# bhavyageethika/multimodal_autonomous_driving_perception_and_planning

Hardware: AMD Instinct MI355X
Metric: end-to-end frames/sec (1280x720 synthetic) (higher is better)
Workload: dtype f64; 1 GPU; config4: 64 stream(s)/GPU x 1-frame window per step, 1280x720, simulated detection + IoU tracker + 6-state KF + 21-candidate planner, one launch per step, up to 4 consecutive steps in flight; streams_per_gpu=64, window=1, graph=False, taggers=False, allgather_track_tables=False, fused_step=True, overlapped_steps=4, steps_per_library_call=8, parallelism=stream-sharded x1

## Files before the change

### include/avhot.h

```cpp
#ifndef AVHOT_H
#define AVHOT_H

#include <stddef.h>
#include <stdint.h>

#ifdef __cplusplus
extern "C" {
#endif

#define AV_VERSION 102

enum {
    AV_OK = 0,
    AV_EINVAL = -1,
    AV_EHIP = -2,
    AV_ENODEV = -3,
    AV_ESTATE = -4,
    AV_ENOMEM = -5
};

typedef struct av_ctx av_ctx;
typedef void* av_stream_t;

int av_version(void);
// ... 73 lines not shown
int av_pack_tracks(av_ctx* ctx, av_stream_t stream, int n_streams, int n_frames, int tcap, int frame_lo, int n_sel,
                   int stream0, int frame0, const av_track_row* snap, const int32_t* snap_n, const int32_t* frame_count, void* wire);

int av_comm_unique_id(void* id128);
int av_comm_create(av_ctx* ctx, const void* id128, int rank, int world, void** comm);
int av_comm_destroy(void* comm);
int av_allgather_tracks(av_ctx* ctx, void* comm, av_stream_t stream, const void* send, void* recv, size_t bytes_per_rank);

typedef struct {
    double dt;
    double process_noise;
    double measurement_noise;
} av_kf_cfg;

#define AV_KF_STATE_DOUBLES 48
#define AV_VSTATE_DOUBLES 12
int av_kf_reset(av_ctx* ctx, av_stream_t stream, int n_streams, double* kf_state);
int av_kf_step(av_ctx* ctx, av_stream_t stream, const av_kf_cfg* cfg, int n_streams, int n_frames,
               const double* z, const uint8_t* mode, double* kf_state, double* out_state,
               double* plan_state);

typedef struct {
    double planning_horizon;
    double dt;
    int32_t num_samples;
    int32_t reserved;
    double w_lateral, w_velocity, w_acceleration, w_curvature;
} av_planner_cfg;

#define AV_WP_DOUBLES 6
int av_planner_configure(av_ctx* ctx, const av_planner_cfg* cfg);
int av_planner_dims(const av_ctx* ctx, int* n_points, int* n_candidates);
int av_planner_launch_shape(int n_points, int n_candidates, int n_states, int extra, int32_t out[4]);
int av_planner_plan(av_ctx* ctx, av_stream_t stream, int n_states, const double* state,
                    const double* ref_path, int n_ref, const double* obstacles, int n_obs,
                    double* waypoints, double* cost, int32_t* order);

int av_planner_plan_each(av_ctx* ctx, av_stream_t stream, int n_states, const double* state,
                         const double* ref_path, const int32_t* n_ref, int rcap, int ref_stride,
                         const double* obstacles, const int32_t* n_obs, int ocap,
                         double* waypoints, double* cost, int32_t* order);

int av_planner_plan_moving(av_ctx* ctx, av_stream_t stream, int n_states, const double* state,
                           const double* ref_path, const int32_t* n_ref, int rcap, int ref_stride,
                           const double* obstacles, const int32_t* n_obs, int ocap,
                           double* waypoints, double* cost, int32_t* order);

typedef struct {
    double x_center, x_scale;
    double y_far, y_scale;
    double radius[16];
} av_obstacle_cfg;
int av_track_obstacles(av_ctx* ctx, av_stream_t stream, const av_obstacle_cfg* cfg, int n_states, int tcap,
                       const av_track_row* snap, const int32_t* snap_n, const double* plan_state,
                       int ocap, double* obstacles, int32_t* n_obs);
int av_track_obstacles_moving(av_ctx* ctx, av_stream_t stream, const av_obstacle_cfg* cfg, double frame_rate, int n_states,
                              int tcap, const av_track_row* snap, const int32_t* snap_n, const double* plan_state,
                              int ocap, double* obstacles, int32_t* n_obs);

int av_dets_to_tracker(av_ctx* ctx, av_stream_t stream, int n_frames, int max_det, const int32_t* src_n,
                       const float* src_box, const float* src_conf, const int32_t* src_cls, const int32_t* class_map,
                       int n_map, int dcap, int32_t* det_n, int32_t* det_box, int32_t* det_cls, double* det_conf,
                       int32_t* dropped);

int av_lane_paths(av_ctx* ctx, av_stream_t stream, const av_obstacle_cfg* cfg, int n_streams, int h, int w, int n_points,
                  const double* poly, const int32_t* pts, const int32_t* info, const double* plan_state, int ref_stride,
// ... 224 lines not shown
```

### multimodal_autonomous_driving_perception_and_planning_amd/_native.py

```python
import ctypes as C
import os

_HERE = os.path.dirname(os.path.abspath(__file__))
LIB_PATH = os.path.join(_HERE, "libavhot.so")

c_i32p = C.POINTER(C.c_int32)
c_f64p = C.POINTER(C.c_double)
vp = C.c_void_p


class TrackerCfg(C.Structure):
    _fields_ = [("iou_threshold", C.c_double), ("max_age", C.c_int32), ("min_hits", C.c_int32),
                ("trajectory_length", C.c_int32)]


class KfCfg(C.Structure):
    _fields_ = [("dt", C.c_double), ("process_noise", C.c_double), ("measurement_noise", C.c_double)]


class PlannerCfg(C.Structure):
    _fields_ = [("planning_horizon", C.c_double), ("dt", C.c_double), ("num_samples", C.c_int32),
                ("reserved", C.c_int32), ("w_lateral", C.c_double), ("w_velocity", C.c_double),
                ("w_acceleration", C.c_double), ("w_curvature", C.c_double)]

# ... 69 lines not shown
    ("av_side_stream", C.c_int, [vp, C.POINTER(vp)]),
    ("av_fork", C.c_int, [vp, vp]),
    ("av_join", C.c_int, [vp, vp]),
    ("av_graph_begin", C.c_int, [vp, vp]),
    ("av_graph_end", C.c_int, [vp, vp, C.POINTER(C.c_int)]),
    ("av_graph_launch", C.c_int, [vp, C.c_int, vp]),
    ("av_graph_destroy", C.c_int, [vp, C.c_int]),
    ("av_event_create", C.c_int, [C.POINTER(vp)]),
    ("av_event_destroy", C.c_int, [vp]),
    ("av_event_record", C.c_int, [vp, vp]),
    ("av_event_elapsed_ms", C.c_int, [vp, vp, C.POINTER(C.c_float)]),
    ("av_stream_sync", C.c_int, [vp]),
    ("av_stream_sync_spin", C.c_int, [vp]),
    ("av_host_alloc", C.c_int, [C.POINTER(vp), C.c_size_t]),
    ("av_host_free", C.c_int, [vp]),
    ("av_copy_h2d", C.c_int, [vp, vp, C.c_size_t, vp]),
    ("av_copy_d2h", C.c_int, [vp, vp, C.c_size_t, vp, C.c_int]),
    ("av_simdet_generate", C.c_int, [vp, vp, C.c_int, C.c_int, C.c_int, C.c_int, C.c_int, vp, vp, vp, vp, vp, vp]),
    ("av_tracker_state_bytes", C.c_size_t, [C.c_int, C.c_int]),
    ("av_tracker_reset", C.c_int, [vp, vp, C.c_int, C.c_int, C.c_int, vp]),
    ("av_tracker_update", C.c_int, [vp, vp, C.POINTER(TrackerCfg), C.c_int, C.c_int, C.c_int, vp, vp, vp, vp,
                                    C.c_int, vp, vp, vp, vp]),
    ("av_wire_table_bytes", C.c_size_t, [C.c_int]),
    ("av_pack_tracks", C.c_int, [vp, vp, C.c_int, C.c_int, C.c_int, C.c_int, C.c_int, C.c_int, C.c_int, vp, vp, vp, vp]),
    ("av_comm_unique_id", C.c_int, [vp]),
    ("av_comm_create", C.c_int, [vp, vp, C.c_int, C.c_int, C.POINTER(vp)]),
    ("av_comm_destroy", C.c_int, [vp]),
    ("av_allgather_tracks", C.c_int, [vp, vp, vp, vp, vp, C.c_size_t]),
    ("av_kf_reset", C.c_int, [vp, vp, C.c_int, vp]),
    ("av_kf_step", C.c_int, [vp, vp, C.POINTER(KfCfg), C.c_int, C.c_int, vp, vp, vp, vp, vp]),
    ("av_planner_configure", C.c_int, [vp, C.POINTER(PlannerCfg)]),
    ("av_planner_dims", C.c_int, [vp, C.POINTER(C.c_int), C.POINTER(C.c_int)]),
    ("av_planner_launch_shape", C.c_int, [C.c_int, C.c_int, C.c_int, C.c_int, c_i32p]),
    ("av_planner_plan", C.c_int, [vp, vp, C.c_int, vp, vp, C.c_int, vp, C.c_int, vp, vp, vp]),
    ("av_planner_plan_each", C.c_int, [vp, vp, C.c_int, vp, vp, vp, C.c_int, C.c_int, vp, vp, C.c_int, vp, vp, vp]),
    ("av_track_obstacles", C.c_int, [vp, vp, C.POINTER(ObstacleCfg), C.c_int, C.c_int, vp, vp, vp, C.c_int, vp, vp]),
    ("av_planner_plan_moving", C.c_int, [vp, vp, C.c_int, vp, vp, vp, C.c_int, C.c_int, vp, vp, C.c_int, vp, vp, vp]),
    ("av_track_obstacles_moving", C.c_int, [vp, vp, C.POINTER(ObstacleCfg), C.c_double, C.c_int, C.c_int, vp, vp, vp, C.c_int, vp,
                                            vp]),
    ("av_dets_to_tracker", C.c_int, [vp, vp, C.c_int, C.c_int, vp, vp, vp, vp, vp, C.c_int, C.c_int, vp, vp, vp, vp, vp]),
    ("av_lane_paths", C.c_int, [vp, vp, C.POINTER(ObstacleCfg), C.c_int, C.c_int, C.c_int, C.c_int, vp, vp, vp, vp, C.c_int,
                                C.c_int, vp, vp, vp]),
    ("av_hot_step", C.c_int, [vp, vp, C.POINTER(TrackerCfg), C.POINTER(KfCfg)] + [C.c_int] * 5 + [vp] * 17 + [vp, C.c_int, C.c_int]),
    ("av_hot_step_fits", C.c_int, [vp, C.c_int, C.c_int, C.c_int, C.c_int]),
    ("av_hot_steps_seq", C.c_int, [vp, C.c_int, vp, C.POINTER(TrackerCfg), C.POINTER(KfCfg)] + [C.c_int] * 5 + [vp] * 7 +
     [C.c_int, C.c_int, vp, C.c_int, C.c_int]),
    ("av_hot_step_seq", C.c_int, [vp, vp, C.POINTER(TrackerCfg), C.POINTER(KfCfg)] + [C.c_int] * 5 + [vp] * 17 +
     [vp, C.c_int, C.c_int, vp, C.c_int, C.c_int]),
    ("av_planner_generate", C.c_int, [vp, vp, C.c_int, vp, vp, vp, vp]),
    ("av_planner_evaluate", C.c_int, [vp, vp, C.c_int, C.c_int, vp, vp, C.c_int, vp, C.c_int, vp]),
    ("av_planner_evaluate_moving", C.c_int, [vp, vp, C.c_int, C.c_int, vp, vp, C.c_int, vp, C.c_int, vp]),
    ("av_lane_workspace_bytes", C.c_size_t, [C.c_int, C.c_int, C.c_int, C.c_int]),
    ("av_lane_workspace_init", C.c_int, [vp, vp, C.c_int, C.c_int, C.c_int, C.c_int, vp]),
    ("av_lane_workspace_view", C.c_int, [C.c_int, C.c_int, C.c_int, C.c_int, C.c_int, C.POINTER(C.c_size_t),
                                         C.POINTER(C.c_size_t)]),
    ("av_raster_draw", C.c_int, [vp, vp, C.c_int, C.c_int, C.c_int, vp, vp, C.c_int, vp, vp, C.c_int]),
    ("av_bev_prim_cap", C.c_int, [vp, C.c_int, C.c_int]),
    ("av_bev_build", C.c_int, [vp, vp, vp, C.c_int, C.c_int, C.c_int, C.c_int, C.c_int, vp, vp, vp, vp, vp, vp, vp, C.c_int, vp]),
    ("av_i420_to_bgr", C.c_int, [vp, vp, C.c_int, C.c_int, C.c_int, vp, vp]),
    ("av_resize_into", C.c_int, [vp, vp, vp, C.c_int, C.c_int, vp, C.c_int, C.c_int, C.c_int, C.c_int]),
    ("av_synth_frames", C.c_int, [vp, vp, C.c_int, C.c_int, C.c_int, C.c_int, C.c_int, vp]),
    ("av_maneuver_reset", C.c_int, [vp, vp, C.c_int, vp]),
    ("av_interaction_state_bytes", C.c_size_t, [C.c_int]),
    ("av_interaction_reset", C.c_int, [vp, vp, C.c_int, C.c_int, vp]),
    ("av_interaction_detect", C.c_int, [vp, vp, vp, C.c_int, C.c_int, C.c_int, vp, vp, vp, vp, vp, vp, vp, vp]),
    ("av_maneuver_detect", C.c_int, [vp, vp, C.c_int, C.c_int, vp, vp, vp, vp]),
# ... 151 lines not shown
```

### multimodal_autonomous_driving_perception_and_planning_amd/csrc/planner.hip

```cpp
#include "common.h"

#include <cmath>



namespace {

struct PlanParams {
    int n, n_lat, C;
    double dt, H;
    double w_lat, w_vel, w_acc, w_curv;
    const double *t, *alpha, *q, *dtd, *lat;
    double atq[20];
};

static const double ATAN_Q[20] = {
    -0x1.5555555555549p-2, 0x1.99999999979b9p-3,  -0x1.24924923e22b4p-3, 0x1.c71c718e5a102p-4,
    -0x1.745d120df88fbp-4, 0x1.3b1362fc35ab5p-4,  -0x1.110deef367776p-4, 0x1.e1b3c8d50e91fp-5,
    -0x1.ae2c7119eb922p-5, 0x1.81fdd2525246ap-5,  -0x1.56daf4786fd80p-5, 0x1.2575526b2309ap-5,
    -0x1.d168e01adf666p-6, 0x1.462cc26bda000p-6,  -0x1.8055065b73333p-7, 0x1.693bd6b79999ap-8,
    -0x1.fdf4e15cccccdp-10, 0x1.f224118000000p-12, -0x1.2568700000000p-14, 0x1.2ed799999999ap-18,
};

__device__ __forceinline__ double atan2_fast(double y, double x, const double (&Q)[20]) {
// ... 63 lines not shown
    tile[(size_t)(n - 1) * 6 + 2] = n > 1 ? tile[(size_t)(n - 2) * 6 + 2] : h0;
}
__device__ __forceinline__ double ref_path_term(double w_lat, const double* ref, int n_ref, double x, double y) {
    double md = INFINITY;
    for (int r = 0; r < n_ref; ++r) {
        const double dx = ref[2 * r] - x, dy = ref[2 * r + 1] - y;
        const double dd = sqrt(dx * dx + dy * dy);
        md = dd < md ? dd : md;
    }
    return w_lat * (md * md);
}
template <bool MOVING>
__device__ __forceinline__ void add_obstacle_penalty(double& sum, const double* o, double x, double y, double tw) {
    double ox = o[0], oy = o[1];
    const double rad = o[2];
    if constexpr (MOVING) ox = ox + o[3] * tw, oy = oy + o[4] * tw;
    const double ex = x - ox, ey = y - oy;
    const double dist = sqrt(ex * ex + ey * ey);
    if (dist < rad * 2.0) sum = sum + 1000.0 * (rad * 2.0 - dist);
    else if (dist < rad * 4.0) sum = sum + 10.0 / (dist - rad + 0.1);
}
__device__ __forceinline__ void rank_and_store(const double* cc, int C, int c, int f, double* __restrict__ cost,
                                               int32_t* __restrict__ order) {
    const double mine = cc[c];
    int rank = 0;
    for (int o2 = 0; o2 < C; ++o2) {
        const double v = cc[o2];
        rank += (v < mine || (v == mine && o2 < c)) ? 1 : 0;
    }
    cost[(size_t)f * C + c] = mine;
    order[(size_t)f * C + rank] = c;
}

struct PlanNoHook {
    __device__ __forceinline__ void operator()(int) const {}
};

struct PlanLists {
    const double* ref; int n_ref;
    const double* obs; int n_obs;
};
struct PlanShared {
    static constexpr int OSTRIDE = 3;
    static constexpr bool MOVING = false;
    const double* ref; int n_ref;
    const double* obs; int n_obs;
    __device__ __forceinline__ PlanLists at(int) const { return PlanLists{ref, n_ref, obs, n_obs}; }
    __device__ __forceinline__ bool has_ref(int) const { return n_ref > 0; }
};
template <int OS>
struct PlanEachT {
    static constexpr int OSTRIDE = OS;
    static constexpr bool MOVING = OS == 5;
    const double* ref; const int32_t* n_ref;
    const double* obs; const int32_t* n_obs;
    int rcap, ref_stride, ocap;
    __device__ __forceinline__ int path_points(int pth) const {
        const int k = n_ref[pth] > rcap ? rcap : n_ref[pth];
        return k < 2 ? 0 : k;
    }
    __device__ __forceinline__ bool has_ref(int f) const { return ref && path_points(f / ref_stride) > 0; }
    __device__ __forceinline__ PlanLists at(int f) const {
        f = __builtin_amdgcn_readfirstlane(f);
        PlanLists l{nullptr, 0, nullptr, 0};
        if (ref) {
            const int pth = f / ref_stride;
            l.n_ref = path_points(pth);
            l.ref = ref + (size_t)pth * rcap * 2;
        }
        if (obs) {
            const int k = n_obs[f];
            l.n_obs = k < 0 ? 0 : (k > ocap ? ocap : k);
            l.obs = obs + (size_t)f * ocap * OS;
        }
        return l;
    }
};
using PlanEach = PlanEachT<3>;
using PlanEachMoving = PlanEachT<5>;

template <int G, int NW, class Hook = PlanNoHook, class Lists = PlanShared>
__device__ __forceinline__ void plan_block_lists(const PlanParams& p, int f0, int n_states, const double* __restrict__ state,
                                                 const Lists lists, double* __restrict__ wp, double* __restrict__ cost,
                                                 int32_t* __restrict__ order, double* sm, int state_f0 = -1, int rot = 0,
                                                 Hook after1 = Hook()) {
    const int n = p.n, C = p.C;
    const int sd = state_f0 < 0 ? 0 : state_f0 - f0;
    double* vs = sm;
    double* base = vs + (size_t)G * 3 * n * 2;
    double* trig = base + even_up(G * 3 * 3);
    double* costs = trig + G * 8;
    double* stage_all = costs + 3 * even_up(G * C);
    const int CS = even_up(G * C);

    const int tid = threadIdx.x, lane = tid & 63;
    double* stage = stage_all + (size_t)(tid >> 6) * n * 6;
    const int wid = ((tid >> 6) + NW - rot) % NW;
    constexpr int P = G * 3;
    static_assert(NW >= 2, "the heading terms take the last wave");

    auto bcast = [&](double x, int i) {
        const unsigned lo = (unsigned)__builtin_amdgcn_readlane((int)(unsigned)__double_as_longlong(x), i);
        const unsigned hi = (unsigned)__builtin_amdgcn_readlane((int)(unsigned)((unsigned long long)__double_as_longlong(x) >> 32), i);
        return __longlong_as_double((long long)(((unsigned long long)hi << 32) | lo));
    };
    auto terms = [&](double v0, double dv, int i, double& v, double& vdt, double& velt, double& acct) {
        v = blend_velocity(v0, dv, p.alpha[i]);
        vdt = v * p.dt;
        velt = velocity_term(p.w_vel, v);
        acct = 0.0;
        if (i > 0)
            acct = acceleration_term(p.w_acc, v, blend_velocity(v0, dv, p.alpha[i - 1]), p.dtd[i]);
    };
    auto cost_chains = [&](double velt, double acct, unsigned long long hasm, double* b) {
        double sv = 0.0;
#pragma unroll
        for (int i = 0; i < 64; ++i)
            if (i < n) sv = sv + bcast(velt, i);
        double run = sv, sa = 0.0;
#pragma unroll
        for (int i = 1; i < 64; ++i)
            if (i < n && ((hasm >> i) & 1ull)) {
                const double term = bcast(acct, i);
                run = run + term, sa = sa + term;
            }
        if (lane == 0) b[0] = sv, b[1] = sa, b[2] = run;
    };

    const bool fast = n <= 64 && P <= NW;
    double k_velt = 0.0, k_acct = 0.0;
    unsigned long long k_has = 0;
    bool k_live = false;
    if (fast) {
        if (wid < P) {
            const int g = wid / 3, k = wid - g * 3, f = f0 + g;
            if (f < n_states) {
                const double v0 = state[(size_t)(f + sd) * 4 + 3];
                const double dv = target_speed(k) - v0;
                double* o = vs + ((size_t)(g * 3 + k) * n) * 2;
                double v = 0.0, vdt = 0.0;
                bool has = false;
                if (lane < n) terms(v0, dv, lane, v, vdt, k_velt, k_acct), has = lane > 0 && p.dtd[lane] > 0.0;
                k_has = __ballot(has), k_live = true;
                double sacc = 0.0, my_s = 0.0;
#pragma unroll
                for (int i = 1; i < 64; ++i)
                    if (i < n) {
                        sacc = sacc + bcast(vdt, i);
                        my_s = lane == i ? sacc : my_s;
                    }
                if (lane < n) o[2 * lane] = v, o[2 * lane + 1] = my_s;
            }
        }
    } else {
        for (int pr = wid; pr < P; pr += NW) {
            const int g = pr / 3, k = pr - g * 3, f = f0 + g;
            if (f >= n_states) continue;
            const double v0 = state[(size_t)(f + sd) * 4 + 3];
            const double dv = target_speed(k) - v0;
            double* o = vs + ((size_t)(g * 3 + k) * n) * 2;
            double* b = base + (g * 3 + k) * 3;
            double* tv = stage;
            for (int i = lane; i < n; i += 64) {
                double v, vdt, velt, acct;
                terms(v0, dv, i, v, vdt, velt, acct);
                o[2 * i] = v, tv[i] = vdt, tv[n + i] = velt, tv[2 * n + i] = acct;
            }
            wave_lds_fence();
            if (lane == 0) {
                double sacc = 0.0, sv = 0.0;
                o[1] = 0.0;
                sv = sv + tv[n];
                for (int i = 1; i < n; ++i) {
                    sacc = sacc + tv[i];
                    o[2 * i + 1] = sacc;
                    sv = sv + tv[n + i];
                }
                double run = sv, sa = 0.0;
                for (int i = 1; i < n; ++i) {
                    if (p.dtd[i] > 0.0) {
                        const double term = tv[2 * n + i];
                        run = run + term, sa = sa + term;
                    }
                }
                b[0] = sv, b[1] = sa, b[2] = run;
            }
            wave_lds_fence();
        }
    }
    if (wid == NW - 1 && lane < 2 * G) {
        const int g = lane >> 1, f = f0 + g;
        if (f < n_states) {
            const double h0 = state[(size_t)(f + sd) * 4 + 2];
            double* tg = trig + g * 8;
            double sn, cs;
            if (lane & 1) {
                sincos(h0 + 1.5707963267948966, &sn, &cs);
                tg[4] = cs, tg[5] = sn;
            } else {
                sincos(h0, &sn, &cs);
                tg[0] = state[(size_t)(f + sd) * 4 + 0], tg[1] = state[(size_t)(f + sd) * 4 + 1];
                tg[2] = cs, tg[3] = sn, tg[6] = h0;
            }
        }
    }
    __syncthreads();
    if (k_live) cost_chains(k_velt, k_acct, k_has, base + wid * 3);
    after1(wid);

    const double q_l = lane < n ? p.q[lane] : 0.0, q_l1 = lane + 1 < n ? p.q[lane + 1] : 0.0, t_l = lane < n ? p.t[lane] : 0.0;
    for (int j = fast ? (wid - P % NW + NW) % NW : wid; j < G * C; j += NW) {
        const int g = j / C, c = j - g * C, f = f0 + g;
        if (f >= n_states) continue;
        const PlanLists ls = lists.at(f);
        const double* ref = ls.ref;
        const double* obs = ls.obs;
        const int n_ref = ls.n_ref, n_obs = ls.n_obs;
        const bool extra = n_ref > 0 || n_obs > 0;
        const int li = c / 3, k = c - li * 3;
        const double df = p.lat[li];
        const double* tg = trig + g * 8;
        const PlanFrame fr{tg[0], tg[1], tg[2], tg[3], tg[4], tg[5]};
        const double h0 = tg[6];
        const double* o = vs + ((size_t)(g * 3 + k) * n) * 2;

        for (int i = lane; i < n; i += 64) {
            const double v = o[2 * i], s = o[2 * i + 1];
            const bool first = i == lane;
            double x, y, hd = 0.0;
            fr.point(s, df * (first ? q_l : p.q[i]), x, y);
            if (i < n - 1) {
                double x1, y1;
                fr.point(o[2 * i + 3], df * (first ? q_l1 : p.q[i + 1]), x1, y1);
                hd = atan2_fast(y1 - y, x1 - x, p.atq);
            }
            double* w = stage + (size_t)i * 6;
            w[0] = x, w[1] = y, w[2] = hd, w[3] = v, w[4] = first ? t_l : p.t[i], w[5] = 0.0;
        }
        wave_lds_fence();
        double lat_sum = 0.0, curv_sum = 0.0, obs_sum = 0.0;
        for (int i = lane; i < n; i += 64) {
            double* w = stage + (size_t)i * 6;
            double curv = 0.0;
            if (i > 0 && i < n - 1) w[5] = curv = tile_curvature(stage, i, p.dt);
            curv_sum += p.w_curv * (curv * curv);
            const double x = w[0], y = w[1];
            if (n_ref > 0) lat_sum += ref_path_term(p.w_lat, ref, n_ref, x, y);
            for (int q = 0; q < n_obs; ++q)
                add_obstacle_penalty<Lists::MOVING>(obs_sum, obs + Lists::OSTRIDE * q, x, y, w[4]);
        }
        wave_lds_fence();
        if (lane == 0) tile_last_heading(stage, n, h0);
        curv_sum = wave_sum_dpp(curv_sum);
        if (extra) lat_sum = wave_sum_dpp(lat_sum), obs_sum = wave_sum_dpp(obs_sum);
        if (lane == 0) costs[g * C + c] = lat_sum, costs[CS + g * C + c] = curv_sum, costs[2 * CS + g * C + c] = obs_sum;
        wave_lds_fence();
        if (wp) {
            const double2* src = reinterpret_cast<const double2*>(stage);
            double2* dst = reinterpret_cast<double2*>(wp + ((size_t)f * C + c) * n * 6);
            for (int q = lane; q < n * 3; q += 64) dst[q] = src[q];
        }
        wave_lds_fence();
    }
    __syncthreads();

    for (int idx = tid; idx < G * C; idx += NW * 64) {
        const int g = idx / C, c = idx - g * C, k = c % 3;
        const double* b = base + (g * 3 + k) * 3;
        const bool with_ref = lists.has_ref(f0 + g < n_states ? f0 + g : f0);
        const double va = with_ref ? (costs[idx] + b[0]) + b[1] : b[2];
        const double total = (va + costs[CS + idx]) + costs[2 * CS + idx];
        costs[idx] = total;
    }
    __syncthreads();
    for (int idx = tid; idx < G * C; idx += NW * 64) {
        const int g = idx / C, c = idx - g * C, f = f0 + g;
        if (f >= n_states) continue;
        rank_and_store(costs + g * C, C, c, f, cost, order);
    }
}

template <int G, int NW, class Hook = PlanNoHook>
__device__ __forceinline__ void plan_block(const PlanParams& p, int f0, int n_states, const double* state, const double* ref, int n_ref,
                                           const double* obs, int n_obs, double* wp, double* cost, int32_t* order, double* sm,
                                           int state_f0 = -1, int rot = 0, Hook after1 = Hook()) {
    plan_block_lists<G, NW, Hook, PlanShared>(p, f0, n_states, state, PlanShared{ref, n_ref, obs, n_obs}, wp, cost, order, sm, state_f0,
                                              rot, after1);
}

template <int G, int NW, class Lists = PlanShared>
__global__ void __launch_bounds__(NW * 64) planner_kernel(PlanParams p, int n_states, const double* __restrict__ state, Lists lists,
                                                          double* __restrict__ wp, double* __restrict__ cost,
                                                          int32_t* __restrict__ order) {
    extern __shared__ __attribute__((aligned(16))) double sm[];
    plan_block_lists<G, NW, PlanNoHook, Lists>(p, blockIdx.x * G, n_states, state, lists, wp, cost, order, sm);
}

template <int FPW, bool EXTRA, class Lists = PlanShared>
__global__ void __launch_bounds__(256) planner_wave_kernel(PlanParams p, int n_states,
                                                           const double* __restrict__ state, Lists lists,
                                                           double* __restrict__ wp, double* __restrict__ cost,
                                                           int32_t* __restrict__ order) {
    extern __shared__ __attribute__((aligned(16))) double sm[];
    const int n = p.n, C = p.C;
    const int lane = threadIdx.x & 63, wid = threadIdx.x >> 6;
    double* vs = sm + wid * wave_lds_doubles(FPW, n, C);
    double* stage = vs + (size_t)FPW * 3 * n * 2;
    double* costs = stage + RING_DOUBLES;
    double* base = costs + even_up(FPW * C);
    double* trig = base + FPW * 3 * 4;
    const long long gw = (long long)blockIdx.x * 4 + wid;
    const long long f0l = gw * FPW;
    if (f0l >= n_states) return;
    const int f0 = (int)f0l;
    const int nf = (n_states - f0) < FPW ? (n_states - f0) : FPW;

    const bool in = lane < n;
    const int li_c = in ? lane : n - 1;
    const int ln_c = (lane + 1 < n) ? lane + 1 : n - 1;
    const int lp_c = li_c > 0 ? li_c - 1 : 0;
    const double q_i = p.q[li_c], q_n = p.q[ln_c], t_i = p.t[li_c];
    const double al_i = p.alpha[li_c], al_p = p.alpha[lp_c], dtd_i = p.dtd[li_c];
    const double lat_l = p.lat[lane < p.n_lat ? lane : 0];
    double st_x[FPW], st_y[FPW], st_h[FPW], st_v[FPW];
#pragma unroll
    for (int g = 0; g < FPW; ++g) {
        const double4 sv4 = reinterpret_cast<const double4*>(state)[f0 + (g < nf ? g : 0)];
        st_x[g] = sv4.x, st_y[g] = sv4.y, st_h[g] = sv4.z, st_v[g] = sv4.w;
// ... 387 lines not shown
        lat[nl - 1] = 3.5;
    }
    AV_HIP(hipSetDevice(ctx->device));
    if (ctx->d_ptab) {
        AV_HIP(hipFree(ctx->d_ptab));
        ctx->d_ptab = nullptr;
    }
    AV_HIP(hipMalloc(&ctx->d_ptab, tab.size() * sizeof(double)));
    AV_HIP(hipMemcpy(ctx->d_ptab, tab.data(), tab.size() * sizeof(double), hipMemcpyHostToDevice));
    ctx->pcfg = *cfg;
    ctx->n_points = n, ctx->n_lat = nl, ctx->n_cand = 3 * nl;
    ctx->planner_ready = true;
    return AV_OK;
}

int av_planner_dims(const av_ctx* ctx, int* n_points, int* n_candidates) {
    AV_REQUIRE(ctx && n_points && n_candidates, AV_EINVAL, "av_planner_dims: null argument");
    AV_REQUIRE(ctx->planner_ready, AV_ESTATE, "av_planner_dims: call av_planner_configure first");
    *n_points = ctx->n_points, *n_candidates = ctx->n_cand;
    return AV_OK;
}

int av_planner_launch_shape(int n_points, int n_candidates, int n_states, int extra, int32_t out[4]) {
    AV_REQUIRE(out, AV_EINVAL, "av_planner_launch_shape: null argument");
    AV_REQUIRE(n_points >= 1 && n_points <= 256 && n_candidates >= 3 && n_candidates <= 192 && n_candidates % 3 == 0, AV_EINVAL,
               "av_planner_launch_shape: %d waypoints, %d candidates: not a configuration av_planner_configure accepts", n_points,
               n_candidates);
    AV_REQUIRE(n_states > 0, AV_EINVAL, "av_planner_launch_shape: n_states must be > 0");
    const PlanLaunch<PlanShared> l = planner_plan<PlanShared>(n_points, n_candidates, n_states, extra != 0);
    out[0] = l.inst->wave, out[1] = l.inst->G, out[2] = l.inst->NW, out[3] = (int32_t)l.lds;
    return AV_OK;
}

int av_planner_plan(av_ctx* ctx, av_stream_t stream, int n_states, const double* state, const double* ref_path,
                    int n_ref, const double* obstacles, int n_obs, double* waypoints, double* cost, int32_t* order) {
    AV_REQUIRE(ctx && state && cost && order, AV_EINVAL, "av_planner_plan: null argument");
    AV_REQUIRE(ctx->planner_ready, AV_ESTATE, "av_planner_plan: call av_planner_configure first");
    AV_REQUIRE(n_states > 0, AV_EINVAL, "av_planner_plan: n_states must be > 0");
    AV_REQUIRE(n_ref >= 0 && n_obs >= 0 && (n_ref == 0 || ref_path) && (n_obs == 0 || obstacles), AV_EINVAL,
               "av_planner_plan: ref_path/obstacles pointer missing");
    AV_REQUIRE(n_ref != 1, AV_EINVAL, "av_planner_plan: a reference path needs >= 2 points (set_reference_path ignores shorter)");
    return plan_dispatch(ctx, as_stream(stream), n_states, state, PlanShared{ref_path, n_ref, obstacles, n_obs}, n_ref > 0 || n_obs > 0,
                         waypoints, cost, order, "av_planner_plan");
}

int av_planner_plan_each(av_ctx* ctx, av_stream_t stream, int n_states, const double* state, const double* ref_path,
                         const int32_t* n_ref, int rcap, int ref_stride, const double* obstacles, const int32_t* n_obs, int ocap,
                         double* waypoints, double* cost, int32_t* order) {
    return plan_each_launch<3>(ctx, stream, n_states, state, ref_path, n_ref, rcap, ref_stride, obstacles, n_obs, ocap, waypoints, cost,
                               order, "av_planner_plan_each");
}

int av_planner_plan_moving(av_ctx* ctx, av_stream_t stream, int n_states, const double* state, const double* ref_path,
                           const int32_t* n_ref, int rcap, int ref_stride, const double* obstacles, const int32_t* n_obs, int ocap,
                           double* waypoints, double* cost, int32_t* order) {
    return plan_each_launch<5>(ctx, stream, n_states, state, ref_path, n_ref, rcap, ref_stride, obstacles, n_obs, ocap, waypoints, cost,
                               order, "av_planner_plan_moving");
}

}

#endif
```

### multimodal_autonomous_driving_perception_and_planning_amd/csrc/step.hip

```cpp
#define AVHOT_DEVICE_ONLY
#include "simdet.hip"
#include "tracker.hip"
#include "kf.hip"
#include "planner.hip"
#undef AVHOT_DEVICE_ONLY

namespace {

struct StepArgs {
    int S, h, w, dcap, tcap;
    av_tracker_cfg tcfg;
    av_kf_cfg kcfg;
    PlanParams pp;
    int32_t* frame_count; const SimRow* tab; const double* cdf;
    int32_t *det_n, *det_box, *det_cls; double* det_conf; int32_t* det_status;
    unsigned char* trk_state; av_track_row* snap; int32_t* snap_n; int32_t* det2trk;
    const double* z; double *kf_state, *vstate, *plan_state;
    double *wp, *cost; int32_t* order;
    uint8_t* wire; int stream0, frame0;
    int* flags; int seq, spin, fence, stage_off;
};

constexpr int STEP_NW = 8;

__device__ __host__ inline int flag_fault(int S) { return 64 * S; }
__device__ __host__ inline int flag_base(int S) { return 64 * S + 32; }
__device__ __host__ inline int flag_stats(int S) { return 65 * S + 32; }
struct StepClock {
    unsigned long long t;
    bool on;
    unsigned long long* acc;
    __device__ void start(const StepArgs& a, int role);
    __device__ void mark(int k) {
        if (!on) return;
        const unsigned long long n = __builtin_amdgcn_s_memrealtime();
        atomicAdd(acc + k, n - t);
        t = n;
    }
};

__device__ void StepClock::start(const StepArgs& a, int role) {
    on = a.flags && (a.fence & 8) && threadIdx.x == 0;
    if (!on) return;
    acc = reinterpret_cast<unsigned long long*>(a.flags + flag_stats(a.S)) + role * 16;
    t = __builtin_amdgcn_s_memrealtime();
    atomicAdd(acc + 15, 1ull);
}

__device__ __forceinline__ bool seq_enter(const StepArgs& a, int slot, int* go) {
    if (threadIdx.x == 0) {
        int ok = 0;
        int* const counter = a.flags + 32 * slot;
        int* const fault = a.flags + flag_fault(a.S);
        const int want = a.seq, spin = a.spin;
        for (int n = 0; n <= spin; ++n) {
            if ((int)((unsigned)__hip_atomic_load(counter, __ATOMIC_RELAXED, __HIP_MEMORY_SCOPE_AGENT) - (unsigned)want) >= 0) { ok = 1; break; }
            if ((n & 255) == 255 && __hip_atomic_load(fault, __ATOMIC_RELAXED, __HIP_MEMORY_SCOPE_AGENT) != 0) break;
        }
        if (!ok) atomicOr(a.flags + flag_fault(a.S), 1);
        if (ok && (a.fence & 8) && a.seq != 0) {
            const unsigned long long tp = __hip_atomic_load(reinterpret_cast<unsigned long long*>(a.flags + 32 * slot + 2), __ATOMIC_RELAXED,
                                                            __HIP_MEMORY_SCOPE_AGENT);
            const unsigned long long now = __builtin_amdgcn_s_memrealtime();
            unsigned long long* acc = reinterpret_cast<unsigned long long*>(a.flags + flag_stats(a.S)) + (slot & 1) * 16;
            if (now > tp) atomicAdd(acc + 8, now - tp), atomicAdd(acc + 9, 1ull);
        }
        *go = ok;
    }
    __syncthreads();
    if (!*go) return false;
    if (a.fence & 1) __builtin_amdgcn_fence(__ATOMIC_ACQUIRE, "agent");
    return true;
}
__device__ __forceinline__ void seq_leave(const StepArgs& a, int slot) {
    if (a.fence & 2) __builtin_amdgcn_fence(__ATOMIC_RELEASE, "agent");
    if (a.fence & 8)
        __hip_atomic_store(reinterpret_cast<unsigned long long*>(a.flags + 32 * slot + 2), __builtin_amdgcn_s_memrealtime(), __ATOMIC_RELAXED,
                           __HIP_MEMORY_SCOPE_AGENT);
    __hip_atomic_store(a.flags + 32 * slot, (int)((unsigned)a.seq + 1u), __ATOMIC_RELAXED, __HIP_MEMORY_SCOPE_AGENT);
}
__device__ __forceinline__ void fetch_record(const void* src, void* dst_lds, int n8, int first, int end, bool coherent) {
    unsigned long long* g = const_cast<unsigned long long*>(reinterpret_cast<const unsigned long long*>(src));
    unsigned long long* l = reinterpret_cast<unsigned long long*>(dst_lds);
    if ((int)threadIdx.x < first || (int)threadIdx.x >= end) return;
    for (int i = (int)threadIdx.x - first; i < n8; i += end - first)
        l[i] = coherent ? __hip_atomic_load(g + i, __ATOMIC_RELAXED, __HIP_MEMORY_SCOPE_AGENT) : g[i];
}

template <int PW>
__global__ void __launch_bounds__(PW * 64) hot_step_kernel(StepArgs a) {
    extern __shared__ __attribute__((aligned(16))) unsigned char smem[];
    __shared__ int go, fc_stage;
    __shared__ __attribute__((aligned(16))) double kf_stage[AV_KF_STATE_DOUBLES + 2];
    __shared__ __attribute__((aligned(32))) double kf_start[4];
    __shared__ __attribute__((aligned(16))) double kf_carry[KF_CARRY_DOUBLES];
    __shared__ int kf_tail;
    __shared__ __attribute__((aligned(16))) int d_box[8 * 4];
    __shared__ __attribute__((aligned(16))) double d_conf[8], d_area[8], z_stage[4];
    __shared__ int d_cls[8], d_n[1];
    const int tid = threadIdx.x;
    const bool seq = a.flags != nullptr;
    if ((int)blockIdx.x < a.S) {
        if (PW > STEP_NW && tid >= STEP_NW * 64) return;
        const int s = blockIdx.x;
        StepClock ck;
        ck.start(a, 0);
        int fc_before = 0;
        if (tid == 0) {
            fc_before = seq ? (int)((unsigned)a.flags[flag_base(a.S) + s] + (unsigned)a.seq) : a.frame_count[s];
            fc_stage = fc_before;
            simdet_frame<true>(0, 0, 0, a.h, a.w, a.dcap, &fc_stage, a.tab, a.cdf, d_n, d_box, d_cls, d_conf,
                               a.det_status ? a.det_status + s : nullptr);
            for (int i = 0; i < a.dcap; ++i)
                d_area[i] = (double)(d_box[4 * i + 2] - d_box[4 * i]) * (double)(d_box[4 * i + 3] - d_box[4 * i + 1]);
        }
        ck.mark(0);
        if (seq && !seq_enter(a, 2 * s, &go)) return;
        ck.mark(1);
        unsigned char* stage = smem + a.stage_off;
        int fc0 = 0;
        if (seq && tid == 0) fc0 = __hip_atomic_load(a.frame_count + s, __ATOMIC_RELAXED, __HIP_MEMORY_SCOPE_AGENT);
        fetch_record(a.trk_state + (size_t)s * state_bytes(a.tcap, a.tcfg.trajectory_length), stage,
                     (HDR_INTS * 4 + a.tcap * (int)sizeof(av_track_row)) / 8, 64, STEP_NW * 64, seq);
        if (tid == 0) {
            if (seq) {
                if (fc0 != fc_before) atomicOr(a.flags + flag_fault(a.S), 2);
                __hip_atomic_store(a.frame_count + s, fc_stage, __ATOMIC_RELAXED, __HIP_MEMORY_SCOPE_AGENT);
            } else {
                a.frame_count[s] = fc_stage;
            }
        }
        if (seq) __builtin_amdgcn_s_waitcnt(0x0F70);
        __syncthreads();
        ck.mark(2);
        if (tid < a.dcap) {
            reinterpret_cast<int4*>(a.det_box)[(size_t)s * a.dcap + tid] = reinterpret_cast<const int4*>(d_box)[tid];
            a.det_cls[(size_t)s * a.dcap + tid] = d_cls[tid];
            a.det_conf[(size_t)s * a.dcap + tid] = d_conf[tid];
            if (tid == 0) a.det_n[s] = d_n[0];
        }
        tracker_body<false, 8, STEP_NW>(a.tcfg, 1, a.dcap, d_n, d_box, d_cls, d_conf, a.tcap, a.trk_state, a.snap, a.snap_n,
                                        a.det2trk, 1, s, smem, 0xFEDCBA9876543210ull, stage, seq, 0,
                                        seq ? a.flags + 32 * (2 * s) : nullptr, (int)((unsigned)a.seq + 1u), (a.fence & 8) != 0, d_area);
        ck.mark(3);
        if (a.wire) {
            __syncthreads();
            if (tid < a.tcap)
                wire_put(a.wire + (size_t)s * (AV_WIRE_HDR_BYTES + (size_t)a.tcap * AV_WIRE_ROW_BYTES), tid, a.snap_n[s], a.tcap,
                         a.snap + (size_t)s * a.tcap, a.stream0 + s, a.frame0 + fc_stage);
        }
    } else {
        const int s = blockIdx.x - a.S;
        StepClock ck;
        ck.start(a, 1);
        if (tid < 4) z_stage[tid] = a.z[(size_t)s * 4 + tid];
        if (seq && !seq_enter(a, 2 * s + 1, &go)) return;
        ck.mark(1);
        double *vs = a.vstate + (size_t)s * AV_VSTATE_DOUBLES, *ps = a.plan_state + (size_t)s * 4;
        if (tid < 64) {
            double* rec = a.kf_state + (size_t)s * AV_KF_STATE_DOUBLES;
            fetch_record(rec, kf_stage, AV_KF_STATE_DOUBLES, 0, 64, seq);
            __builtin_amdgcn_fence(__ATOMIC_RELEASE, "workgroup", "local");
            __builtin_amdgcn_wave_barrier();
            __builtin_amdgcn_fence(__ATOMIC_ACQUIRE, "workgroup", "local");
            ck.mark(2);
            const bool separable = kf_axis_chain1(a.kcfg, z_stage, kf_stage, kf_start, kf_carry, tid);
            if (tid == 0) {
                kf_tail = separable;
                if (!separable) {
                    kf_dense_stream_lds(a.kcfg, 0, 1, z_stage, nullptr, kf_stage, vs, kf_start);
                    *reinterpret_cast<double4*>(ps) = *reinterpret_cast<const double4*>(kf_start);
                }
            }
            __builtin_amdgcn_fence(__ATOMIC_RELEASE, "workgroup", "local");
            __builtin_amdgcn_wave_barrier();
            __builtin_amdgcn_fence(__ATOMIC_ACQUIRE, "workgroup", "local");
            if (tid < AV_KF_STATE_DOUBLES) {
                if (seq)
                    __hip_atomic_store(reinterpret_cast<unsigned long long*>(rec) + tid, (unsigned long long)__double_as_longlong(kf_stage[tid]),
                                       __ATOMIC_RELAXED, __HIP_MEMORY_SCOPE_AGENT);
                else
                    rec[tid] = kf_stage[tid];
            }
        }
        ck.mark(3);
        __syncthreads();
        ck.mark(4);
        constexpr int KF_ROT = 4;
        static_assert(KF_ROT + 3 < PW, "wave 0 must not be a phase-1 pair wave nor the heading wave (task wave PW - 1)");
        if (seq && tid < 64) {
            __builtin_amdgcn_s_waitcnt(0x0F70);
            if (tid == 0) seq_leave(a, 2 * s + 1);
        }
        ck.mark(5);
        const bool clocks = seq && (a.fence & 8);
        auto tail = [&](int task_wave) {
            if (task_wave != 0 || !kf_tail) return;
            const unsigned long long t0 = clocks ? __builtin_amdgcn_s_memrealtime() : 0ull;
            kf_axis_tail1(a.kcfg, kf_stage, kf_carry, vs, ps, tid & 63);
            if (clocks && (tid & 63) == 0)
                atomicAdd(reinterpret_cast<unsigned long long*>(a.flags + flag_stats(a.S)) + 16 + 7, __builtin_amdgcn_s_memrealtime() - t0);
        };
        plan_block<1, PW>(a.pp, s, a.S, kf_start, nullptr, 0, nullptr, 0, a.wp, a.cost, a.order, reinterpret_cast<double*>(smem), 0, KF_ROT,
                          tail);
        ck.mark(6);
    }
}

}

static size_t hot_step_tracker_lds(int dcap, int tcap, int& stage_off) {
    static_assert(STEP_NW == 8, "tracker_lds_bytes sizes the replica kernel's eight column waves");
    const size_t lds_t = (tracker_lds_bytes(tcap, dcap, 1, true, 0) + 15) & ~size_t(15);
    stage_off = (int)lds_t;
    return lds_t + HDR_INTS * 4 + (size_t)tcap * sizeof(av_track_row);
}

static size_t hot_step_static_lds(const void* kernel) {
    hipFuncAttributes fa{};
    return hipFuncGetAttributes(&fa, kernel) == hipSuccess ? (size_t)fa.sharedSizeBytes : (size_t)16384;
}

static int hot_step_shape(const av_ctx* ctx, int n_streams, size_t lds_t, int depth, size_t& lds_out, int& pw_out) {
    static const size_t lds_static16 = hot_step_static_lds(reinterpret_cast<const void*>(hot_step_kernel<16>));
    static const size_t lds_static8 = hot_step_static_lds(reinterpret_cast<const void*>(hot_step_kernel<8>));
    const char* pwe = getenv("AVHOT_STEP_PW");
    int pw = pwe && atoi(pwe) == 8 ? 8 : 16;
    size_t lds = 0;
    for (;;) {
        const size_t lds_p = plan_lds_doubles(1, ctx->n_points, ctx->n_cand, pw) * 8;
        lds = lds_t > lds_p ? lds_t : lds_p;
        const size_t lds_static = pw == 16 ? lds_static16 : lds_static8;
        if (lds + lds_static > 64 * 1024) {
            AV_REQUIRE(pw == 16 && !pwe, AV_EINVAL,
                       "av_hot_step: configuration needs %zu B of dynamic + %zu B of static LDS (limit 65536)", lds, lds_static);
            pw = 8;
            continue;
// ... 139 lines not shown
```

Before: 13.45 million frames/s.

## Run planner cost chains on spare waves beside arc-length waves and prefetch lane tables

When the workgroup has at least 2P+1 waves, the per-candidate cost-chain reductions now run on separate waves concurrently with the arc-length prefix sums, instead of after the first barrier. Per-lane planner tables (alpha, dtd, q, t, lat) are loaded before the sequencing wait so their global loads overlap the KF dependency. The unrolled 64-iteration broadcast loops become 8-wide chunks bounded by n, and the KF tail hook is moved to a wave that has no phase-1 work. Timing stamps and a host query for the wave assignment are also added.

```diff
diff --git a/include/avhot.h b/include/avhot.h
--- a/include/avhot.h
+++ b/include/avhot.h
@@ -129,6 +129,7 @@
 int av_planner_configure(av_ctx* ctx, const av_planner_cfg* cfg);
 int av_planner_dims(const av_ctx* ctx, int* n_points, int* n_candidates);
 int av_planner_launch_shape(int n_points, int n_candidates, int n_states, int extra, int32_t out[4]);
+int av_planner_dealing(int n_points, int nw, int32_t out[24]);
 int av_planner_plan(av_ctx* ctx, av_stream_t stream, int n_states, const double* state,
                     const double* ref_path, int n_ref, const double* obstacles, int n_obs,
                     double* waypoints, double* cost, int32_t* order);
diff --git a/multimodal_autonomous_driving_perception_and_planning_amd/_native.py b/multimodal_autonomous_driving_perception_and_planning_amd/_native.py
--- a/multimodal_autonomous_driving_perception_and_planning_amd/_native.py
+++ b/multimodal_autonomous_driving_perception_and_planning_amd/_native.py
@@ -125,6 +125,7 @@
     ("av_planner_configure", C.c_int, [vp, C.POINTER(PlannerCfg)]),
     ("av_planner_dims", C.c_int, [vp, C.POINTER(C.c_int), C.POINTER(C.c_int)]),
     ("av_planner_launch_shape", C.c_int, [C.c_int, C.c_int, C.c_int, C.c_int, c_i32p]),
+    ("av_planner_dealing", C.c_int, [C.c_int, C.c_int, c_i32p]),
     ("av_planner_plan", C.c_int, [vp, vp, C.c_int, vp, vp, C.c_int, vp, C.c_int, vp, vp, vp]),
     ("av_planner_plan_each", C.c_int, [vp, vp, C.c_int, vp, vp, vp, C.c_int, C.c_int, vp, vp, C.c_int, vp, vp, vp]),
     ("av_track_obstacles", C.c_int, [vp, vp, C.POINTER(ObstacleCfg), C.c_int, C.c_int, vp, vp, vp, C.c_int, vp, vp]),
diff --git a/multimodal_autonomous_driving_perception_and_planning_amd/csrc/planner.hip b/multimodal_autonomous_driving_perception_and_planning_amd/csrc/planner.hip
--- a/multimodal_autonomous_driving_perception_and_planning_amd/csrc/planner.hip
+++ b/multimodal_autonomous_driving_perception_and_planning_amd/csrc/planner.hip
@@ -119,9 +119,16 @@
     order[(size_t)f * C + rank] = c;
 }
 
+enum PlanEvent { PLAN_EV_ARC, PLAN_EV_CHAIN, PLAN_EV_BARRIER1, PLAN_EV_TRAJ, PLAN_EV_BARRIER2 };
 struct PlanNoHook {
     __device__ __forceinline__ void operator()(int) const {}
-};
+    __device__ __forceinline__ void stamp(int, int, int) const {}
+};
+
+__host__ __device__ constexpr bool plan_chains_beside(int P, int NW) { return NW >= 2 * P + 1; }
+__host__ __device__ constexpr int plan_chain_wave(int P, int NW, int pr) { return plan_chains_beside(P, NW) ? P + pr : pr; }
+__host__ __device__ constexpr int plan_first_traj(int P, int NW, int wid) { return (wid - P % NW + NW) % NW; }
+__host__ __device__ constexpr int plan_tail_wave(int P, int NW) { return plan_chains_beside(P, NW) ? P - 1 : NW - 1; }
 
 struct PlanLists {
     const double* ref; int n_ref;
@@ -166,11 +173,24 @@
 using PlanEach = PlanEachT<3>;
 using PlanEachMoving = PlanEachT<5>;
 
+struct PlanLaneTab {
+    double alpha, alpha_p, dtd, q, q1, t, lat;
+};
+__device__ __forceinline__ PlanLaneTab plan_lane_tab(const PlanParams& p, int lane) {
+    const int n = p.n;
+    PlanLaneTab tb;
+    tb.alpha = lane < n ? p.alpha[lane] : 0.0, tb.alpha_p = lane > 0 && lane < n ? p.alpha[lane - 1] : 0.0;
+    tb.dtd = lane < n ? p.dtd[lane] : 0.0;
+    tb.q = lane < n ? p.q[lane] : 0.0, tb.q1 = lane + 1 < n ? p.q[lane + 1] : 0.0, tb.t = lane < n ? p.t[lane] : 0.0;
+    tb.lat = p.lat[lane < p.n_lat ? lane : 0];
+    return tb;
+}
+
 template <int G, int NW, class Hook = PlanNoHook, class Lists = PlanShared>
-__device__ __forceinline__ void plan_block_lists(const PlanParams& p, int f0, int n_states, const double* __restrict__ state,
-                                                 const Lists lists, double* __restrict__ wp, double* __restrict__ cost,
-                                                 int32_t* __restrict__ order, double* sm, int state_f0 = -1, int rot = 0,
-                                                 Hook after1 = Hook()) {
+__device__ __forceinline__ void plan_block_lists(const PlanParams& p, const PlanLaneTab tb, int f0, int n_states,
+                                                 const double* __restrict__ state, const Lists lists, double* __restrict__ wp,
+                                                 double* __restrict__ cost, int32_t* __restrict__ order, double* sm, int state_f0 = -1,
+                                                 int rot = 0, Hook after1 = Hook()) {
     const int n = p.n, C = p.C;
     const int sd = state_f0 < 0 ? 0 : state_f0 - f0;
     double* vs = sm;
@@ -191,52 +211,68 @@
         const unsigned hi = (unsigned)__builtin_amdgcn_readlane((int)(unsigned)((unsigned long long)__double_as_longlong(x) >> 32), i);
         return __longlong_as_double((long long)(((unsigned long long)hi << 32) | lo));
     };
-    auto terms = [&](double v0, double dv, int i, double& v, double& vdt, double& velt, double& acct) {
-        v = blend_velocity(v0, dv, p.alpha[i]);
+    auto terms = [&](double v0, double dv, int i, double al, double alp, double dtdi, double& v, double& vdt, double& velt, double& acct) {
+        v = blend_velocity(v0, dv, al);
         vdt = v * p.dt;
         velt = velocity_term(p.w_vel, v);
         acct = 0.0;
         if (i > 0)
-            acct = acceleration_term(p.w_acc, v, blend_velocity(v0, dv, p.alpha[i - 1]), p.dtd[i]);
+            acct = acceleration_term(p.w_acc, v, blend_velocity(v0, dv, alp), dtdi);
     };
-    auto cost_chains = [&](double velt, double acct, unsigned long long hasm, double* b) {
+    auto cost_chains = [&](double velt, double accz, double* b) {
         double sv = 0.0;
+#pragma unroll 1
+        for (int i0 = 0; i0 < n; i0 += 8) {
 #pragma unroll
-        for (int i = 0; i < 64; ++i)
-            if (i < n) sv = sv + bcast(velt, i);
+            for (int i = 0; i < 8; ++i) sv = sv + bcast(velt, i0 + i);
+        }
         double run = sv, sa = 0.0;
+#pragma unroll 1
+        for (int i0 = 0; i0 < n; i0 += 8) {
 #pragma unroll
-        for (int i = 1; i < 64; ++i)
-            if (i < n && ((hasm >> i) & 1ull)) {
-                const double term = bcast(acct, i);
+            for (int i = 0; i < 8; ++i) {
+                const double term = bcast(accz, i0 + i);
                 run = run + term, sa = sa + term;
             }
+        }
         if (lane == 0) b[0] = sv, b[1] = sa, b[2] = run;
     };
 
     const bool fast = n <= 64 && P <= NW;
+    constexpr bool beside = plan_chains_beside(P, NW);
     double k_velt = 0.0, k_acct = 0.0;
-    unsigned long long k_has = 0;
     bool k_live = false;
     if (fast) {
-        if (wid < P) {
-            const int g = wid / 3, k = wid - g * 3, f = f0 + g;
+        const int pr = wid < P ? wid : (beside && wid < 2 * P ? wid - P : -1);
+        if (pr >= 0) {
+            const int g = pr / 3, k = pr - g * 3, f = f0 + g;
             if (f < n_states) {
                 const double v0 = state[(size_t)(f + sd) * 4 + 3];
                 const double dv = target_speed(k) - v0;
-                double* o = vs + ((size_t)(g * 3 + k) * n) * 2;
                 double v = 0.0, vdt = 0.0;
-                bool has = false;
-                if (lane < n) terms(v0, dv, lane, v, vdt, k_velt, k_acct), has = lane > 0 && p.dtd[lane] > 0.0;
-                k_has = __ballot(has), k_live = true;
-                double sacc = 0.0, my_s = 0.0;
+                if (lane < n) {
+                    terms(v0, dv, lane, tb.alpha, tb.alpha_p, tb.dtd, v, vdt, k_velt, k_acct);
+                    k_acct = lane > 0 && tb.dtd > 0.0 ? k_acct : 0.0;
+                }
+                if (wid < P) {
+                    double* o = vs + ((size_t)pr * n) * 2;
+                    const double sterm = lane > 0 ? vdt : 0.0;
+                    double sacc = 0.0, my_s = 0.0;
+#pragma unroll 1
+                    for (int i0 = 0; i0 < n; i0 += 8) {
 #pragma unroll
-                for (int i = 1; i < 64; ++i)
-                    if (i < n) {
-                        sacc = sacc + bcast(vdt, i);
-                        my_s = lane == i ? sacc : my_s;
+                        for (int i = 0; i < 8; ++i) {
+                            sacc = sacc + bcast(sterm, i0 + i);
+                            my_s = lane == i0 + i ? sacc : my_s;
+                        }
                     }
-                if (lane < n) o[2 * lane] = v, o[2 * lane + 1] = my_s;
+                    if (lane < n) o[2 * lane] = v, o[2 * lane + 1] = my_s;
+                    k_live = !beside;
+                    after1.stamp(PLAN_EV_ARC, wid, 0);
+                } else {
+                    cost_chains(k_velt, k_acct, base + pr * 3);
+                    after1.stamp(PLAN_EV_CHAIN, wid, 0);
+                }
             }
         }
     } else {
@@ -250,7 +286,7 @@
             double* tv = stage;
             for (int i = lane; i < n; i += 64) {
                 double v, vdt, velt, acct;
-                terms(v0, dv, i, v, vdt, velt, acct);
+                terms(v0, dv, i, p.alpha[i], i > 0 ? p.alpha[i - 1] : 0.0, p.dtd[i], v, vdt, velt, acct);
                 o[2 * i] = v, tv[i] = vdt, tv[n + i] = velt, tv[2 * n + i] = acct;
             }
             wave_lds_fence();
@@ -291,12 +327,16 @@
             }
         }
     }
+    after1.stamp(PLAN_EV_BARRIER1, wid, 0);
     __syncthreads();
-    if (k_live) cost_chains(k_velt, k_acct, k_has, base + wid * 3);
+    if (k_live) {
+        cost_chains(k_velt, k_acct, base + wid * 3);
+        after1.stamp(PLAN_EV_CHAIN, wid, 0);
+    }
     after1(wid);
 
-    const double q_l = lane < n ? p.q[lane] : 0.0, q_l1 = lane + 1 < n ? p.q[lane + 1] : 0.0, t_l = lane < n ? p.t[lane] : 0.0;
-    for (int j = fast ? (wid - P % NW + NW) % NW : wid; j < G * C; j += NW) {
+    const double q_l = tb.q, q_l1 = tb.q1, t_l = tb.t;
+    for (int j = fast ? plan_first_traj(P, NW, wid) : wid; j < G * C; j += NW) {
         const int g = j / C, c = j - g * C, f = f0 + g;
         if (f >= n_states) continue;
         const PlanLists ls = lists.at(f);
@@ -305,7 +345,7 @@
         const int n_ref = ls.n_ref, n_obs = ls.n_obs;
         const bool extra = n_ref > 0 || n_obs > 0;
         const int li = c / 3, k = c - li * 3;
-        const double df = p.lat[li];
+        const double df = readlane_f64(tb.lat, li);
         const double* tg = trig + g * 8;
         const PlanFrame fr{tg[0], tg[1], tg[2], tg[3], tg[4], tg[5]};
         const double h0 = tg[6];
@@ -348,7 +388,9 @@
             for (int q = lane; q < n * 3; q += 64) dst[q] = src[q];
         }
         wave_lds_fence();
-    }
+        after1.stamp(PLAN_EV_TRAJ, wid, j / NW);
+    }
+    after1.stamp(PLAN_EV_BARRIER2, wid, 0);
     __syncthreads();
 
     for (int idx = tid; idx < G * C; idx += NW * 64) {
@@ -368,11 +410,11 @@
 }
 
 template <int G, int NW, class Hook = PlanNoHook>
-__device__ __forceinline__ void plan_block(const PlanParams& p, int f0, int n_states, const double* state, const double* ref, int n_ref,
-                                           const double* obs, int n_obs, double* wp, double* cost, int32_t* order, double* sm,
-                                           int state_f0 = -1, int rot = 0, Hook after1 = Hook()) {
-    plan_block_lists<G, NW, Hook, PlanShared>(p, f0, n_states, state, PlanShared{ref, n_ref, obs, n_obs}, wp, cost, order, sm, state_f0,
-                                              rot, after1);
+__device__ __forceinline__ void plan_block(const PlanParams& p, const PlanLaneTab tb, int f0, int n_states, const double* state,
+                                           const double* ref, int n_ref, const double* obs, int n_obs, double* wp, double* cost,
+                                           int32_t* order, double* sm, int state_f0 = -1, int rot = 0, Hook after1 = Hook()) {
+    plan_block_lists<G, NW, Hook, PlanShared>(p, tb, f0, n_states, state, PlanShared{ref, n_ref, obs, n_obs}, wp, cost, order, sm,
+                                              state_f0, rot, after1);
 }
 
 template <int G, int NW, class Lists = PlanShared>
@@ -380,7 +422,8 @@
                                                           double* __restrict__ wp, double* __restrict__ cost,
                                                           int32_t* __restrict__ order) {
     extern __shared__ __attribute__((aligned(16))) double sm[];
-    plan_block_lists<G, NW, PlanNoHook, Lists>(p, blockIdx.x * G, n_states, state, lists, wp, cost, order, sm);
+    plan_block_lists<G, NW, PlanNoHook, Lists>(p, plan_lane_tab(p, threadIdx.x & 63), blockIdx.x * G, n_states, state, lists, wp, cost,
+                                               order, sm);
 }
 
 template <int FPW, bool EXTRA, class Lists = PlanShared>
@@ -834,6 +877,20 @@
     return AV_OK;
 }
 
+int av_planner_dealing(int n_points, int nw, int32_t out[24]) {
+    AV_REQUIRE(out, AV_EINVAL, "av_planner_dealing: null argument");
+    AV_REQUIRE(n_points >= 1 && n_points <= 256, AV_EINVAL, "av_planner_dealing: %d waypoints not in [1,256]", n_points);
+    AV_REQUIRE(nw == 2 || nw == 4 || nw == 8 || nw == 16, AV_EINVAL, "av_planner_dealing: %d waves: the workgroups have 2, 4, 8 or 16", nw);
+    constexpr int P = 3;
+    const bool fast = n_points <= 64 && P <= nw;
+    out[0] = !fast ? 0 : (plan_chains_beside(P, nw) ? 2 : 1);
+    out[1] = plan_tail_wave(P, nw);
+    for (int pr = 0; pr < P; ++pr) out[2 + pr] = fast ? plan_chain_wave(P, nw, pr) : pr % nw;
+    out[5] = out[6] = out[7] = 0;
+    for (int w = 0; w < 16; ++w) out[8 + w] = w >= nw ? -1 : (fast ? plan_first_traj(P, nw, w) : w);
+    return AV_OK;
+}
+
 int av_planner_plan(av_ctx* ctx, av_stream_t stream, int n_states, const double* state, const double* ref_path,
                     int n_ref, const double* obstacles, int n_obs, double* waypoints, double* cost, int32_t* order) {
     AV_REQUIRE(ctx && state && cost && order, AV_EINVAL, "av_planner_plan: null argument");
diff --git a/multimodal_autonomous_driving_perception_and_planning_amd/csrc/step.hip b/multimodal_autonomous_driving_perception_and_planning_amd/csrc/step.hip
--- a/multimodal_autonomous_driving_perception_and_planning_amd/csrc/step.hip
+++ b/multimodal_autonomous_driving_perception_and_planning_amd/csrc/step.hip
@@ -47,6 +47,47 @@
     atomicAdd(acc + 15, 1ull);
 }
 
+enum StepPlanClock {
+    PCK_ARC = 16,
+    PCK_CHAIN = 26,
+    PCK_BARRIER1 = 27,
+    PCK_BARRIER2_PAIR = 28,
+    PCK_BARRIER2 = 29,
+    PCK_END = 30,
+    PCK_TRAJ_TAIL = 4,
+    PCK_TRAJ_W0 = 10,
+};
+struct StepPlanHook {
+    const StepArgs& a;
+    const double *kf_stage, *kf_carry;
+    double *vs, *ps;
+    const int* kf_tail;
+    const unsigned long long* t0;
+    bool clocks;
+    int tail_wave, chain0_wave;
+    __device__ __forceinline__ void put(int slot) const {
+        atomicAdd(reinterpret_cast<unsigned long long*>(a.flags + flag_stats(a.S)) + slot, __builtin_amdgcn_s_memrealtime() - *t0);
+    }
+    __device__ __forceinline__ void stamp(int ev, int wid, int round) const {
+        if (!clocks || (threadIdx.x & 63) != 0) return;
+        const bool w0 = threadIdx.x == 0;
+        if (ev == PLAN_EV_ARC && wid == 0) put(PCK_ARC);
+        if (ev == PLAN_EV_CHAIN && wid == chain0_wave) put(PCK_CHAIN);
+        if (ev == PLAN_EV_BARRIER1 && w0) put(PCK_BARRIER1);
+        if (ev == PLAN_EV_BARRIER2 && w0) put(PCK_BARRIER2);
+        if (ev == PLAN_EV_BARRIER2 && wid == 0) put(PCK_BARRIER2_PAIR);
+        if (ev == PLAN_EV_TRAJ && round < 3 && w0) put(PCK_TRAJ_W0 + round);
+        if (ev == PLAN_EV_TRAJ && round < 3 && wid == tail_wave) put(PCK_TRAJ_TAIL + round);
+    }
+    __device__ __forceinline__ void operator()(int task_wave) const {
+        if (task_wave != tail_wave || !*kf_tail) return;
+        const unsigned long long t = clocks ? __builtin_amdgcn_s_memrealtime() : 0ull;
+        kf_axis_tail1(a.kcfg, kf_stage, kf_carry, vs, ps, threadIdx.x & 63);
+        if (clocks && (threadIdx.x & 63) == 0)
+            atomicAdd(reinterpret_cast<unsigned long long*>(a.flags + flag_stats(a.S)) + 16 + 7, __builtin_amdgcn_s_memrealtime() - t);
+    }
+};
+
 __device__ __forceinline__ bool seq_enter(const StepArgs& a, int slot, int* go) {
     if (threadIdx.x == 0) {
         int ok = 0;
@@ -95,6 +136,7 @@
     __shared__ __attribute__((aligned(32))) double kf_start[4];
     __shared__ __attribute__((aligned(16))) double kf_carry[KF_CARRY_DOUBLES];
     __shared__ int kf_tail;
+    __shared__ unsigned long long plan_t0;
     __shared__ __attribute__((aligned(16))) int d_box[8 * 4];
     __shared__ __attribute__((aligned(16))) double d_conf[8], d_area[8], z_stage[4];
     __shared__ int d_cls[8], d_n[1];
@@ -154,6 +196,7 @@
         StepClock ck;
         ck.start(a, 1);
         if (tid < 4) z_stage[tid] = a.z[(size_t)s * 4 + tid];
+        const PlanLaneTab ptab = plan_lane_tab(a.pp, tid & 63);
         if (seq && !seq_enter(a, 2 * s + 1, &go)) return;
         ck.mark(1);
         double *vs = a.vstate + (size_t)s * AV_VSTATE_DOUBLES, *ps = a.plan_state + (size_t)s * 4;
@@ -184,25 +227,22 @@
             }
         }
         ck.mark(3);
+        if (ck.on) plan_t0 = ck.t;
         __syncthreads();
         ck.mark(4);
-        constexpr int KF_ROT = 4;
-        static_assert(KF_ROT + 3 < PW, "wave 0 must not be a phase-1 pair wave nor the heading wave (task wave PW - 1)");
+        constexpr int KF_ROT = 2;
+        static_assert(plan_chains_beside(3, PW) && (PW - KF_ROT) % PW >= 2 * 3 && (PW - KF_ROT) % PW < PW - 1,
+                      "wave 0 must have no phase-1 work: no pair's arc length or cost chains, nor the heading terms (task wave PW - 1)");
         if (seq && tid < 64) {
             __builtin_amdgcn_s_waitcnt(0x0F70);
             if (tid == 0) seq_leave(a, 2 * s + 1);
         }
         ck.mark(5);
-        const bool clocks = seq && (a.fence & 8);
-        auto tail = [&](int task_wave) {
-            if (task_wave != 0 || !kf_tail) return;
-            const unsigned long long t0 = clocks ? __builtin_amdgcn_s_memrealtime() : 0ull;
-            kf_axis_tail1(a.kcfg, kf_stage, kf_carry, vs, ps, tid & 63);
-            if (clocks && (tid & 63) == 0)
-                atomicAdd(reinterpret_cast<unsigned long long*>(a.flags + flag_stats(a.S)) + 16 + 7, __builtin_amdgcn_s_memrealtime() - t0);
-        };
-        plan_block<1, PW>(a.pp, s, a.S, kf_start, nullptr, 0, nullptr, 0, a.wp, a.cost, a.order, reinterpret_cast<double*>(smem), 0, KF_ROT,
-                          tail);
+        const StepPlanHook hook{a, kf_stage, kf_carry, vs, ps, &kf_tail, &plan_t0, seq && (a.fence & 8), plan_tail_wave(3, PW),
+                                plan_chain_wave(3, PW, 0)};
+        plan_block<1, PW>(a.pp, ptab, s, a.S, kf_start, nullptr, 0, nullptr, 0, a.wp, a.cost, a.order, reinterpret_cast<double*>(smem), 0, KF_ROT,
+                          hook);
+        if (hook.clocks && tid == 0) hook.put(PCK_END);
         ck.mark(6);
     }
 }
```

Result: no change. 13.60 million frames/s (median of 6 runs) (+1.2%).
